# david8862/tf-keras-speech-commands

Measured on AMD Instinct MI355X. Metric: 1 s@16 kHz clips/sec train-step, simple_cnn bs4096, 1/2/4/8 MI355X; eval top-1, higher is better.
Workload: dtype f32; 1 GPU; configs[1]: simple_cnn train step = featurize(f32 1 s @16 kHz) + fwd + bwd + Adam, 36 logits (background + 35 words), batch 4096 per GPU; global_batch=4096, parallelism=dp1, gradient_exchange=none (one rank), rccl_ranks=0, library_build=ed8bfb18a7f8

## Files before the change

### tf-keras-speech-commands_amd/csrc/kws_cnn_shape.h

```cpp
#pragma once
#include <algorithm>
#include <cstddef>
#include <cstdint>

#include "kws.h"

namespace kws {

constexpr int kStatStride = 1024;
constexpr int kMaxStatBlocks = kStatStride;

constexpr int kFuClips = 16;
constexpr int kFuH2 = 7, kFuW2 = 5;
constexpr int kFuH3 = 4, kFuW3 = 3;
constexpr int kFuH4 = 2, kFuW4 = 1;
constexpr int kFuHeadCols = 48;
constexpr int kGrH1 = 2 * kFuH2 + 1, kGrW1 = 2 * kFuW2;

constexpr int kL1MaxTiles = 40;
constexpr int kL1Stage = 12;

constexpr int kDhK = 128;
constexpr int kDhWaves = 8;

// ... 41 lines not shown
    int pmajor = 0;
};

inline ConvGeom geom3x3(int B, int H, int W, int stride)
{
    ConvGeom g;
    g.B = B; g.H = H; g.W = W; g.stride = stride; g.KH = 3; g.KW = 3;
    g.Ho = same_out(H, stride); g.Wo = same_out(W, stride);
    g.pt = same_pad_before(H, 3, stride); g.pl = same_pad_before(W, 3, stride);
    return g;
}
inline ConvGeom geom1x1(int B, int H, int W)
{
    ConvGeom g;
    g.B = B; g.H = H; g.W = W; g.Ho = H; g.Wo = W; g.stride = 1; g.pt = 0; g.pl = 0; g.KH = 1; g.KW = 1;
    return g;
}
inline ConvGeom dense_geom(const CnnDims &d, int B)
{
    ConvGeom g;
    g.B = B; g.H = d.H4; g.W = d.W4; g.Ho = 1; g.Wo = 1; g.stride = 1; g.pt = 0; g.pl = 0; g.KH = d.H4; g.KW = d.W4;
    return g;
}

inline void stat_grid(long M, int C, int &nblk, int &rows)
{
    const int R = 256 / C;
    long want = (M + (long)R * 8 - 1) / ((long)R * 8);
    nblk = (int)std::min<long>(kMaxStatBlocks, std::max<long>(1, want));
    rows = (int)((M + nblk - 1) / nblk);
    nblk = (int)((M + rows - 1) / rows);
}

constexpr int conv_bf16_rt(bool fwd, int CR, int CO) { return (fwd && CO == 128 && CR == 64) ? 3 : 2; }
inline int conv_bf16_pmajor(const ConvGeom &g, bool fwd)
{
    const int P = fwd ? g.Ho * g.Wo : g.H * g.W;
    return (g.KH == 3 && g.KW == 3 && P > 1 && P <= 16) ? 1 : 0;
}

struct DgradClass { int cy, cx, ny, nx; };
struct DgradClasses { DgradClass c[4]; };

struct DgradPlan { DgradClasses cls; int ncls; long max_rows; int mw; };
enum { DGRAD_OK = 0, DGRAD_KERNEL_TOO_LARGE = 1, DGRAD_STRIDE = 2 };
inline int dgrad_plan(const ConvGeom &g, long simds, DgradPlan &p)
{
    if (g.KH > 8 * g.stride || g.KW > 8 * g.stride) return DGRAD_KERNEL_TOO_LARGE;
    DgradClasses &cls = p.cls;
    int ncls = 0;
    long rows[4] = {0, 0, 0, 0}, max_rows = 0;
    for (int cy = 0; cy < g.stride && cy < 2; ++cy)
        for (int cx = 0; cx < g.stride && cx < 2; ++cx) {
            DgradClass c{cy, cx, (g.H - cy + g.stride - 1) / g.stride, (g.W - cx + g.stride - 1) / g.stride};
            if (c.ny <= 0 || c.nx <= 0) continue;
            rows[ncls] = (long)g.B * c.ny * c.nx;
            max_rows = std::max(max_rows, rows[ncls]);
            cls.c[ncls++] = c;
        }
    for (int i = ncls; i < 4; ++i) cls.c[i] = DgradClass{0, 0, 0, 0};
    if (g.stride > 2) return DGRAD_STRIDE;
    int best = 4;
    long best_cost = -1;
    for (int mw = 4; mw >= 1; --mw) {
        long waves = 0;
        for (int i = 0; i < ncls; ++i) waves += ((rows[i] + 15) / 16 + mw - 1) / mw;
        const long cost = ((waves + simds - 1) / simds) * mw;
        if (best_cost < 0 || cost < best_cost) { best_cost = cost; best = mw; }
    }
    p.ncls = ncls; p.max_rows = max_rows; p.mw = best;
    return DGRAD_OK;
}

struct WgradRound { long gx; int spw; };
inline WgradRound wgrad_round(long steps, int gy, long resident, bool deterministic)
{
    const long slots = deterministic ? 1 : std::max<long>(1, resident / gy);
    const long gx_want = std::max<long>(1, std::min<long>(slots, (steps + 4 * 8 - 1) / (4 * 8)));
    const int spw = (int)((steps + 4 * gx_want - 1) / (4 * gx_want));
    const long gx = (steps + 4L * spw - 1) / (4L * spw);
    return WgradRound{gx, spw};
}

struct WgradBf16Round { long nranges; int cpb; };
inline WgradBf16Round wgrad_bf16_round(long nchunk, int ngroups, long resident, bool deterministic)
{
    long nranges = std::max<long>(8, (resident / ngroups) / 8 * 8);
    nranges = std::min<long>(nranges, std::max<long>(8, (nchunk / 4 + 7) / 8 * 8));
    int cpb = (int)((nchunk + nranges - 1) / nranges);
    if (deterministic) { nranges = 8; cpb = (int)nchunk; }
    return WgradBf16Round{nranges, cpb};
}

struct WgradPm {
    unsigned long long pos[9];
    int npos[9];
    int slot0[10];
};

inline bool wgrad_pm_plan(const ConvGeom &g, int max_slots, int min_chunks, WgradPm &pm)
{
    const int P = g.Ho * g.Wo, ntaps = g.KH * g.KW;
    if (P < 1 || P > 16 || ntaps < 1 || ntaps > 9) return false;
    long w[9], wsum = 0;
    int live = 0;
    for (int tap = 0; tap < ntaps; ++tap) {
        const int kh = tap / g.KW, kw = tap % g.KW;
        pm.pos[tap] = 0ull; pm.npos[tap] = 0;
        for (int p = 0; p < P; ++p) {
            const int sy = (p / g.Wo) * g.stride + kh - g.pt, sx = (p % g.Wo) * g.stride + kw - g.pl;
            if (sy < 0 || sy >= g.H || sx < 0 || sx >= g.W) continue;
            pm.pos[tap] |= (unsigned long long)p << (4 * pm.npos[tap]);
            ++pm.npos[tap];
        }
        w[tap] = pm.npos[tap]; wsum += w[tap]; live += w[tap] > 0;
    }
    if (live < 1 || max_slots < live) return false;
    const long nclip = ((long)g.B + 31) / 32, want = (wsum * nclip + 8L * min_chunks - 1) / (8L * min_chunks);
    const int S = (int)(want < live ? live : want > max_slots ? max_slots : want);
    int s[9], total = 0;
    for (int tap = 0; tap < ntaps; ++tap) {
        s[tap] = w[tap] ? (int)((long)S * w[tap] / wsum) : 0;
        if (w[tap] && s[tap] < 1) s[tap] = 1;
        total += s[tap];
    }
    for (; total < S; ++total) {
        int best = -1;
        for (int tap = 0; tap < ntaps; ++tap)
            if (w[tap] && (best < 0 || w[tap] * s[best] > w[best] * s[tap])) best = tap;
        ++s[best];
    }
    for (; total > S; --total) {
        int best = -1;
        for (int tap = 0; tap < ntaps; ++tap)
            if (s[tap] > 1 && (best < 0 || w[tap] * s[best] <= w[best] * s[tap])) best = tap;
        --s[best];
    }
    pm.slot0[0] = 0;
    for (int tap = 0; tap < ntaps; ++tap) pm.slot0[tap + 1] = pm.slot0[tap] + s[tap];
    for (int tap = ntaps + 1; tap < 10; ++tap) pm.slot0[tap] = pm.slot0[ntaps];
    return true;
}

struct L1Grid {
    int cpb, nb;
    int cpw, nbm;
};
inline L1Grid l1_grid(int B)
{
    L1Grid g;
    g.cpb = std::max(1, (B + kMaxStatBlocks - 1) / kMaxStatBlocks); g.nb = (B + g.cpb - 1) / g.cpb;
    g.cpw = std::max(1, (B + 4 * kMaxStatBlocks - 1) / (4 * kMaxStatBlocks)); g.nbm = (B + 4 * g.cpw - 1) / (4 * g.cpw);
    return g;
}

inline unsigned even_grid(int B, int max_blocks) { const int cpb = (B + max_blocks - 1) / max_blocks; return (unsigned)((B + cpb - 1) / cpb); }

struct LiteFrontGrid { int cpw, nblk; };
inline LiteFrontGrid lite_front_grid(int B, int cus, size_t sm)
{
    const int waves = cus * std::max(1, std::min(8, (int)(160 * 1024 / sm)));
    const int cpw = std::max(1, (B + waves - 1) / waves), nblk = (B + cpw - 1) / cpw;
    return LiteFrontGrid{cpw, nblk};
}

inline bool head_bwd_fuses(int K, int C) { return K % 16 == 0 && K <= 128 && C <= 48; }
// ... 3 lines not shown
```

### tf-keras-speech-commands_amd/csrc/kws_model.hip

```cpp
#include <cstdlib>
#include <cstring>
#include <string>
#include <type_traits>
#include <vector>

#include "kws_common.h"
#include "kws_model_types.h"
#include "kws_conv.h"
#include "kws_layers.h"
#include "kws_layer1.h"
#include "kws_layer1_moments.h"
#include "kws_layer1_fast.h"
#include "kws_l1_conv2.h"
#include "kws_conv2_wgrad_fast.h"
#include "kws_lite.h"
#include "kws_lite_f16.h"
#include "kws_infer_fused.h"
#include "kws_conv_group.h"
#include "kws_dense_head.h"
#include "kws_cnn_plan.h"

using namespace kws;

namespace {

struct OverlapHook {
    hipEvent_t ev = nullptr;
    void (*cb)(void *) = nullptr;
    void *user = nullptr;
    int at = 0;
    bool fired = false;
    bool wants(int point) const { return !fired && point == at; }
    int fire(int point, hipStream_t s, bool already_bound = false)
    {
        if (fired || point != at) return KWS_OK;
        fired = true;
        if (ev && !already_bound) KWS_HIP_CHECK(hipEventRecord(ev, s));
        if (cb) cb(user);
        return KWS_OK;
    }
};

#define KWS_TRY_NB(...)               \
    do {                              \
        const int rc__ = (__VA_ARGS__); \
        if (rc__ < 0) return rc__;    \
    } while (0)
#define KWS_TRY(...)                  \
    do {                              \
        if (int rc__ = (__VA_ARGS__)) return rc__; \
    } while (0)

inline CnnDesc cnn_desc(const kws_model *m) { return CnnDesc{m->kind, m->C, m->head_K, m->deterministic, m->d}; }

struct CnnWs {
    float *z[4], *a[4], *d1, *loss_i, *correct_i, *dlogits, *dd1, *da4, *gz[4], *da[3];
    float *dwo[4], *ddw[4];
    float *coef[4];
    __bf16 *wsp[3][6];
    __bf16 *dzp[3];
    double *partial;
    double *moments;
    float *zmax2;
    unsigned char *arg2;
    float *zmax4;
    unsigned char *arg4;
    unsigned char *base;
    size_t bytes;
};

CnnWs carve_cnn(const kws_model *m, int B, bool training, unsigned char *base)
{
    CnnWs w{};
    w.base = base;
    size_t off = 0;
    auto take = [&](size_t nfloats) {
        float *p = reinterpret_cast<float *>(base + off);
        off = al256(off + nfloats * sizeof(float));
        return p;
    };
    const CnnDims &d = m->d;
    const bool lite = m->kind == KWS_SIMPLE_CNN_LITE;
    size_t zs[4], as[4], dws[4];
    for (int i = 0; i < 4; ++i) {
        const CnnStage t = cnn_stage(d, i);
        zs[i] = (size_t)t.Ho * t.Wo * t.Cout;
        as[i] = t.pooled ? (size_t)(t.Ho / 2) * (t.Wo / 2) * t.Cout : zs[i];
        dws[i] = (size_t)t.Ho * t.Wo * t.Cin;
    }
    for (int i = 0; i < 4; ++i) { w.z[i] = take((i == 0 && !lite) ? 0 : zs[i] * B); w.a[i] = take(as[i] * B); }
    for (int i = 0; i < 4; ++i) w.dwo[i] = take(lite ? dws[i] * B : 0);
    w.d1 = take((size_t)B * 128);
    w.loss_i = take(B);
    w.correct_i = take(B);
    for (int i = 0; i < 4; ++i) w.coef[i] = take(6 * 128);
    {
        const size_t wn[3] = {(size_t)9 * 32 * 64, (size_t)9 * 64 * 128, (size_t)d.flat * 128};
        for (int t = 0; t < 3; ++t)
            for (int q = 0; q < 6; ++q) w.wsp[t][q] = reinterpret_cast<__bf16 *>(take(lite ? 0 : (wn[t] + 1) / 2));
    }
    w.partial = reinterpret_cast<double *>(take((size_t)kMaxStatBlocks * 9 * 64 * 2));
    w.moments = reinterpret_cast<double *>(take(2 * kMomCount));
    if (training) {
        w.dlogits = take((size_t)B * m->C);
        w.dd1 = take((size_t)B * 128);
        w.da4 = take((size_t)B * d.flat);
        for (int i = 0; i < 4; ++i) w.gz[i] = take((i == 0 && !lite) ? 0 : zs[i] * B);
        for (int p = 0; p < 3; ++p) w.dzp[p] = reinterpret_cast<__bf16 *>(take(lite ? 0 : (zs[3] * B + 1) / 2));
        for (int i = 0; i < 4; ++i) w.ddw[i] = take(lite ? dws[i] * B : 0);
        for (int i = 0; i < 3; ++i) w.da[i] = take(as[i] * B);
        w.zmax2 = take(lite ? 0 : as[1] * B);
        w.arg2 = reinterpret_cast<unsigned char *>(take(lite ? 0 : (as[1] * B + 3) / 4));
        w.zmax4 = take(lite ? 0 : as[3] * B);
        w.arg4 = reinterpret_cast<unsigned char *>(take(lite ? 0 : (as[3] * B + 3) / 4));
    }
    w.bytes = off;
    return w;
}

BnCoef coef_of(float *base, int C) { return BnCoef{base, base + C, base + 2 * C, base + 3 * C, base + 4 * C, base + 5 * C}; }
static double *acc_set(ModelRes *R, int pass, int layer, unsigned parity) { return R->acc + ((size_t)(pass * 4 + layer) * 2 + (parity & 1u)) * kAccDoubles; }
static int acc_make_clean(ModelRes *R, hipStream_t s)
{
    if (R->acc_dirty) {
        KWS_HIP_CHECK(hipMemsetAsync(R->acc, 0, sizeof(double) * 2 * 4 * 2 * kAccDoubles, s));
        R->acc_dirty = false;
    }
    return KWS_OK;
}

static int infer_coefs(const kws_model *m, const float *params, const float *state, CnnWs &w, hipStream_t s)
{
    BnInferAll a;
    for (int l = 0; l < 4; ++l) {
        a.C[l] = kCh[l + 1];
        a.gamma[l] = params + m->o_g[l]; a.beta[l] = params + m->o_b[l];
        a.mm[l] = state + m->o_mm[l]; a.mv[l] = state + m->o_mv[l];
        a.k[l] = coef_of(w.coef[l], kCh[l + 1]);
    }
    KWS_LAUNCH("bn_infer_coef_all_kernel", bn_infer_coef_all_kernel, dim3(4), dim3(128), 0, s, a);
    return KWS_OK;
}

template <int CR, int CO, int MODE, int EPI>
int launch_gemm(const float *src, const float *w, const float *bias, float *dst, const ConvGeom &g, hipStream_t s)
{
    const long M = (long)g.B * g.Ho * g.Wo;
    static const std::string name = std::string("conv_gemm_fwd<") + std::to_string(CR) + "," +
                                    std::to_string(CO) + ">";
    KWS_LAUNCH(name.c_str(), (conv_gemm_kernel<CR, CO, MODE, EPI>), dim3(blocks_for(M, 64)), dim3(256), 0, s, src, w, bias, dst, g);
    return KWS_OK;
}

static int cu_count() { return device_cus(); }
template <typename K>
static int resident_blocks(K kernel, int threads, size_t smem)
{
    int nb = 0;
    if (hipOccupancyMaxActiveBlocksPerMultiprocessor(&nb, kernel, threads, smem) != hipSuccess || nb < 1) { (void)hipGetLastError(); nb = 1; }
    return nb;
}

template <int CIN, int COUT, int GPB>
int launch_wgrad(const float *x, const float *dz, float *dw, const ConvGeom &g, hipStream_t s, bool deterministic = false,
                 const LossSumJob *job = nullptr)
{
    const float *zp = zero_page();
    if (!zp) return fail(KWS_ERR_NOMEM, "cannot allocate the zero page on this device");
    constexpr int CB = CIN >= 64 ? 64 : CIN;
    constexpr size_t smem = (4 * 64 * 4 + 16 * COUT) * sizeof(float);
    const long M = (long)g.B * g.Ho * g.Wo;
    const int ngroups = g.KH * g.KW * (CIN / CB), gy = (ngroups + GPB - 1) / GPB;
    const long steps = (M + 3) / 4;
    static const int occ = resident_blocks(conv_wgrad_direct_kernel<CIN, COUT, GPB>, 256, smem);
    const WgradRound r = wgrad_round(steps, gy, (long)cu_count() * occ, deterministic);
    static const std::string name = "conv_wgrad<" + std::to_string(CIN) + "," + std::to_string(COUT) + ">";
    KWS_LAUNCH(name.c_str(), (conv_wgrad_direct_kernel<CIN, COUT, GPB>), dim3((unsigned)r.gx + (job ? 1u : 0u), (unsigned)gy), dim3(256), smem,
               s, x, dz, dw, zp, g, r.spw, job ? *job : LossSumJob{});
    return KWS_OK;
}

template <int CIN, int COUT, int TPB, bool DPRE = false, bool XBN = false>
int launch_wgrad_bf16(const float *x, const float *dz, float *dw, const ConvGeom &g, hipStream_t s, __bf16 *const *dz_planes = nullptr,
                      bool deterministic = false, const float *xbn = nullptr, bool pmajor = false)
{
    if (TPB != 1 && g.KW != TPB) return fail(KWS_ERR_UNSUPPORTED, "split-precision weight gradient expects a kernel %d taps wide", TPB);
    const float *zp = zero_page();
    if (!zp) return fail(KWS_ERR_NOMEM, "cannot allocate the zero page on this device");
    constexpr size_t stage = (size_t)3 * 32 * 4 * (TPB * tr_row_words(CIN) + tr_row_words(COUT)), tile = (size_t)CIN * COUT * sizeof(float);
    constexpr size_t smem = stage > tile ? stage : tile;
    if (int rc = ensure_dynamic_lds(reinterpret_cast<const void *>(conv_wgrad_bf16_kernel<CIN, COUT, TPB, DPRE, XBN>), (int)smem)) return rc;
    static const int occ = resident_blocks(conv_wgrad_bf16_kernel<CIN, COUT, TPB, DPRE, XBN>, 256, smem);
    const long M = (long)g.B * g.Ho * g.Wo, nchunk = (M + 31) / 32;
    const int ngroups = g.KH * g.KW / TPB;
    const WgradBf16Round r = wgrad_bf16_round(nchunk, ngroups, (long)cu_count() * occ, deterministic);
    static const std::string name = "conv_wgrad_bf16<" + std::to_string(CIN) + "," + std::to_string(COUT) + ">";
    const Bf16Planes dpl{{DPRE ? dz_planes[0] : nullptr, DPRE ? dz_planes[1] : nullptr, DPRE ? dz_planes[2] : nullptr}};
    if (pmajor && TPB != 1) return fail(KWS_ERR_UNSUPPORTED, "the position-major weight gradient takes one tap per block");
    if constexpr (TPB == 1) {
        if (pmajor) {
            if (int rc = ensure_dynamic_lds(reinterpret_cast<const void *>(conv_wgrad_bf16_kernel<CIN, COUT, 1, DPRE, XBN, true>), (int)smem)) return rc;
            static const int occ_pm = resident_blocks(conv_wgrad_bf16_kernel<CIN, COUT, 1, DPRE, XBN, true>, 256, smem);
            WgradPm pm{};
            if (!wgrad_pm_plan(g, cu_count() * occ_pm / 8, 4, pm))
                return fail(KWS_ERR_UNSUPPORTED, "position-major weight gradient: a %d x %d map on %d block slots", g.Ho, g.Wo, cu_count() * occ_pm);
            KWS_LAUNCH(name.c_str(), (conv_wgrad_bf16_kernel<CIN, COUT, 1, DPRE, XBN, true>), dim3(8u * (unsigned)pm.slot0[ngroups]), dim3(256), smem, s, x,
                       dz, dw, zp, g, 0, 0, dpl, xbn, pm);
            return KWS_OK;
        }
    }
    KWS_LAUNCH(name.c_str(), (conv_wgrad_bf16_kernel<CIN, COUT, TPB, DPRE, XBN>), dim3((unsigned)(r.nranges * ngroups)), dim3(256), smem, s, x, dz, dw,
               zp, g, r.cpb, (int)r.nranges, dpl, xbn);
    return KWS_OK;
}

template <int CR, int CO, int MW, int STRIDE>
int launch_dgrad_mw(const float *dz, const float *w, float *dx, const ConvGeom &g, const DgradClasses &cls, int ncls, long max_rows,
                     hipStream_t s)
{
    static const std::string name = "conv_dgrad<" + std::to_string(CR) + "," + std::to_string(CO) + ">";
    const float *zp = zero_page();
    if (!zp) return fail(KWS_ERR_NOMEM, "cannot allocate the zero page on this device");
    KWS_LAUNCH(name.c_str(), (conv_dgrad_direct_kernel<CR, CO, MW, STRIDE>), dim3(blocks_for(max_rows, 64 * MW), (unsigned)ncls), dim3(256), 0, s,
               dz, w, dx, zp, g, cls);
    return KWS_OK;
}

template <int CR, int CO, int STRIDE>
int launch_dgrad(const float *dz, const float *w, float *dx, const ConvGeom &g, hipStream_t s)
{
    DgradPlan p;
    switch (dgrad_plan(g, 4L * cu_count(), p)) {
    case DGRAD_KERNEL_TOO_LARGE:
        return fail(KWS_ERR_UNSUPPORTED, "kernel %dx%d too large for the dgrad tap masks (at most %d taps per axis)", g.KH, g.KW, 8 * g.stride);
    case DGRAD_STRIDE: return fail(KWS_ERR_UNSUPPORTED, "dgrad is built for strides 1 and 2");
    default: break;
    }
    switch (p.mw) {
    case 1: return launch_dgrad_mw<CR, CO, 1, STRIDE>(dz, w, dx, g, p.cls, p.ncls, p.max_rows, s);
    case 2: return launch_dgrad_mw<CR, CO, 2, STRIDE>(dz, w, dx, g, p.cls, p.ncls, p.max_rows, s);
    case 3: return launch_dgrad_mw<CR, CO, 3, STRIDE>(dz, w, dx, g, p.cls, p.ncls, p.max_rows, s);
    default: return launch_dgrad_mw<CR, CO, 4, STRIDE>(dz, w, dx, g, p.cls, p.ncls, p.max_rows, s);
    }
}

static int g_matrix_precision = 1;
static inline int matrix_prec(const kws_model *m) { return m->matrix_precision >= 0 ? m->matrix_precision : g_matrix_precision; }
static int g_infer_precision = 0;
static inline int infer_prec(const kws_model *m) { return m->infer_precision >= 0 ? m->infer_precision : g_infer_precision; }

template <int CR, int CO, int MODE, int EPI>
int launch_bf16(const char *what, const float *src, __bf16 *const planes[6], const float *bias, float *dst, const ConvGeom &g_in,
                hipStream_t s, double *partial = nullptr, const float *shift = nullptr, __bf16 *const *src_planes = nullptr,
                const float *abn = nullptr)
{
    ConvGeom g = g_in;
    const long M = MODE == MODE_FWD ? (long)g.B * g.Ho * g.Wo : (long)g.B * g.H * g.W;
    if (M >= (1L << 31)) return fail(KWS_ERR_UNSUPPORTED, "%s: %ld rows exceed the kernel's 32-bit row index", what, M);
    g.pmajor = conv_bf16_pmajor(g, MODE == MODE_FWD);
    static const std::string name = std::string(what) + "<" + std::to_string(CR) + "," + std::to_string(CO) + ">";
    const int o = MODE == MODE_FWD ? 3 : 0;
    const Bf16Planes wp{{planes[o], planes[o + 1], planes[o + 2]}};
// ... 264 lines not shown
                       params + m->o_g[0], params + m->o_b[0], state + m->o_mm[0], state + m->o_mv[0], k1, w.a[0], B, d.H0, d.W0, g.cpw, g.nbm, pa);
        } else {
            KWS_LAUNCH("l1m_act_pool_kernel", l1m_act_pool_moments_kernel<false>, dim3(g.nbm), dim3(256), g.smemm, s, feat, kern1, q,
                       params + m->o_g[0], params + m->o_b[0], state + m->o_mm[0], state + m->o_mv[0], k1, w.a[0], B, d.H0, d.W0, g.cpw, g.nbm, pa);
        }
        return KWS_OK;
    }
    if (P.training) {
        KWS_LAUNCH("l1_stats_kernel", l1_stats_kernel<16>, dim3(g.nb), dim3(256), g.smem1, s, feat, kern1, B, d.H0, d.W0, g.cpb, w.partial);
        KWS_TRY(bn_train_coefs(0, g.nb));
    }
    if (P.l1m) KWS_LAUNCH("l1m_act_pool_kernel", l1m_act_pool_kernel, dim3(g.nbm), dim3(256), g.smemm, s, feat, kern1, k1.scale, k1.shift, w.a[0], B,
               d.H0, d.W0, g.cpw);
    else KWS_LAUNCH("l1_act_pool_kernel", l1_act_pool_kernel<16>, dim3(g.nb), dim3(256), g.smem1, s, feat, kern1, k1.scale, k1.shift, w.a[0], B,
               d.H0, d.W0, g.cpb);
    return KWS_OK;
}

int CnnStep::bn_train_coefs(int l, int fused_stat_blocks)
{
    const long M = pixels(l);
    const int C = kCh[l + 1];
    int nblk, rows;
    stat_grid(M, C, nblk, rows);
    if (fused_stat_blocks) nblk = fused_stat_blocks;
    else KWS_LAUNCH(prof_name("channel_stats_kernel", l + 1), channel_stats_kernel, dim3(nblk), dim3(256), 0, s, w.z[l], M, C, rows, w.partial);
    KWS_LAUNCH(prof_name("bn_finalize_train_kernel", l + 1), bn_finalize_train_kernel, dim3(C), dim3(64), 0, s, w.partial, nblk, M, C, params + m->o_g[l],
               params + m->o_b[l], state + m->o_mm[l], state + m->o_mv[l], coef(l));
    return KWS_OK;
}
int CnnStep::bn_act(int l, float rate, float *zm, unsigned char *ag)
{
    const BnCoef k = coef(l);
    const CnnStage t = cnn_stage(d, l);
    const int H = t.Ho, W = t.Wo, C = t.Cout;
    if (t.pooled) {
        const long total = (long)B * (H / 2) * (W / 2) * C;
        KWS_LAUNCH(prof_name("bn_act_pool_kernel", l + 1), bn_act_pool_kernel<true>, dim3(blocks_for(total, 256)), dim3(256), 0, s, w.z[l], k.scale, k.shift,
                   w.a[l], B, H, W, C, rate, slo(), shi(), zm, ag);
    } else {
        const long total = pixels(l) * C;
        KWS_LAUNCH(prof_name("bn_act_pool_kernel", l + 1), bn_act_pool_kernel<false>, dim3(blocks_for(total, 256)), dim3(256), 0, s, w.z[l], k.scale, k.shift,
                           w.a[l], B, H, W, C, rate, slo(), shi());
    }
    return KWS_OK;
}
int CnnStep::bn_bwd_finalize(int l, int nblk)
{
    const int C = kCh[l + 1];
    KWS_LAUNCH(prof_name("bn_bwd_finalize_kernel", l + 1), bn_bwd_finalize_kernel, dim3(C), dim3(64), 0, s, w.partial, nblk, pixels(l), C, params + m->o_g[l],
               grads + m->o_g[l], grads + m->o_b[l], coef(l));
    return KWS_OK;
}
template <bool RELU>
int CnnStep::bn_bwd_apply(int l)
{
    const int C = kCh[l + 1];
    const long total = pixels(l) * C;
    KWS_LAUNCH(prof_name("bn_bwd_apply_kernel", l + 1), bn_bwd_apply_kernel<RELU>, dim3(blocks_for(total, 256)), dim3(256), 0, s, w.z[l], w.gz[l], coef(l),
               params + m->o_g[l], total, C);
    return KWS_OK;
}

int CnnStep::colsum(const char *label, const float *x, long M, int C, float *dst)
{
    int nblk, rows;
    stat_grid(M, C, nblk, rows);
    KWS_LAUNCH(label, channel_stats_kernel, dim3(nblk), dim3(256), 0, s, x, M, C, rows, w.partial);
    KWS_LAUNCH("colsum_finalize_kernel", colsum_finalize_kernel, dim3(C), dim3(256), 0, s, w.partial, nblk, C, dst);
    return KWS_OK;
}
int CnnStep::head_train(const kws_train_args *a, float *stats)
{
    KWS_TRY(run_head(m, B, params, w.d1, w.loss_i, w.correct_i, a->labels, a->class_weights, a->probs, nullptr, w.dlogits, a->grad_scale / (float)B,
                     stats, a->ignore_index, s));
    if (a->forward_event) KWS_HIP_CHECK(hipEventRecord(static_cast<hipEvent_t>(a->forward_event), s));
    return KWS_OK;
}

int CnnStep::dense_fwd() { return launch_gemm<128, 128, MODE_FWD, EPI_BIAS_RELU6>(w.a[3], params + m->o_dk, params + m->o_db, w.d1, dense_geom(d, B), s); }
int CnnStep::dense_bias_grad() { return colsum("channel_stats_kernel.dense", w.dd1, B, 128, grads + m->o_db); }
int CnnStep::dense_wgrad(hipStream_t on, bool det, const LossSumJob *job)
{
    return launch_wgrad<128, 128, 1>(w.a[3], w.dd1, grads + m->o_dk, dense_geom(d, B), on, det, job);
}
int CnnStep::dense_dgrad() { return launch_dgrad<128, 128, 1>(w.dd1, params + m->o_dk, w.da4, dense_geom(d, B), s); }

int CnnCtx::fwd_conv2()
{
    const float *in = w.a[0], *kern = params + m->o_k[1];
    const unsigned nblk = (unsigned)std::min(B, kMaxStatBlocks);
    const Conv2Clip cc = conv2_clip(d, B);
    if (!P.training) {
        const BnCoef k2 = coef(1);
        if (P.bf16) {
            KWS_LAUNCH("conv_fwd_clip_pool_bf16<16,32>", (conv_fwd_clip_bf16_kernel<false, true>), dim3(nblk), dim3(256), cc.smb, s, in, kern, w.a[1], B,
                       d.H1, d.W1, w.partial, kStatStride, k2.scale, k2.shift);
            if (P.fused_tail) KWS_TRY(launch_fused_tail(m, B, params, w, probs, argmax, s));
        } else
            KWS_LAUNCH("conv_fwd_clip_pool<16,32>", (conv_fwd_clip_kernel<32, false, true>), dim3(nblk), dim3(256), cc.sm, s, in, kern, w.a[1], B,
                       d.H1, d.W1, w.partial, kStatStride, k2.scale, k2.shift);
        return KWS_OK;
    }
    if (P.l1_conv2) ;
    else if (P.bf16)
        KWS_LAUNCH("conv_fwd_clip_bf16<16,32>", (conv_fwd_clip_bf16_kernel<true>), dim3(nblk), dim3(256), cc.smb, s, in, kern, w.z[1], B, d.H1,
                   d.W1, w.partial, kStatStride, nullptr, nullptr, P.acc_fwd ? acc_set(R, 0, 1, fpar[1]) : nullptr);
    else
        KWS_LAUNCH("conv_fwd_clip<16,32>", (conv_fwd_clip_kernel<32, true>), dim3(nblk), dim3(256), cc.sm, s, in, kern, w.z[1], B, d.H1, d.W1,
                   w.partial, kStatStride);
    if (hook) KWS_TRY(hook->fire(9, s));
    if (!P.acc_fwd) KWS_TRY(bn_train_coefs(1, (int)nblk));
    if (!P.fuse_pool2) KWS_TRY(bn_act(1, 0.f, P.routed_g2 ? w.zmax2 : nullptr, P.routed_g2 ? w.arg2 : nullptr));
    return KWS_OK;
}

int CnnCtx::fwd_conv3()
{
    const float *in = w.a[1], *kern = params + m->o_k[2];
    const ConvGeom g = geom3x3(B, d.H2, d.W2, 2);
    if (P.bf16 && !P.training) {
        const BnCoef k3 = coef(2);
        KWS_TRY_NB(launch_bf16<32, 64, MODE_FWD, EPI_BN_RELU6>("conv_bf16_fwd_bn", in, w.wsp[0], k3.scale, w.a[2], g, s, nullptr, k3.shift));
        return KWS_OK;
    }
    if (P.bf16 && P.training && !P.prep_in_stats) KWS_HIP_CHECK(hipStreamWaitEvent(s, R->ev[11], 0));
    int fused_stat_blocks = 0;
    if (P.group) {
        if (P.acc_fwd) { const BnAccFwd in2 = acc_in(1, fpar[1]); fused_stat_blocks = launch_group_conv3(m, B, w, s, P.fuse_pool2, &in2, acc_set(R, 0, 2, fpar[2])); }
        else fused_stat_blocks = launch_group_conv3(m, B, w, s, P.fuse_pool2);
        if (fused_stat_blocks < 0) return fused_stat_blocks;
    } else if (P.bf16) {
        fused_stat_blocks = launch_bf16<32, 64, MODE_FWD, EPI_NONE>("conv_bf16_fwd", in, w.wsp[0], nullptr, w.z[2], g, s, P.training ? w.partial : nullptr);
        if (fused_stat_blocks < 0) return fused_stat_blocks;
    } else KWS_TRY(launch_gemm<32, 64, MODE_FWD, EPI_NONE>(in, kern, nullptr, w.z[2], g, s));
    if (hook) KWS_TRY(hook->fire(10, s));
    if (P.training && !P.acc_fwd) KWS_TRY(bn_train_coefs(2, fused_stat_blocks));
    if (!P.a3_on_load) KWS_TRY(bn_act(2, 0.f));
    return KWS_OK;
}

int CnnCtx::fwd_conv4()
{
    const float *in = w.a[2], *kern = params + m->o_k[3];
    const ConvGeom g = geom3x3(B, d.H3, d.W3, 1);
    int fused_stat_blocks = 0;
    if (P.group) {
        if (P.acc_fwd) { const BnAccFwd in3 = acc_in(2, fpar[2]); fused_stat_blocks = launch_group_conv4(m, B, w, s, &in3, acc_set(R, 0, 3, fpar[3])); }
        else fused_stat_blocks = launch_group_conv4(m, B, w, s);
        if (fused_stat_blocks < 0) return fused_stat_blocks;
    } else if (P.bf16) {
        fused_stat_blocks = launch_bf16<64, 128, MODE_FWD, EPI_RELU>("conv_bf16_fwd", P.a3_on_load ? w.z[2] : in, w.wsp[1], nullptr, w.z[3], g, s,
                                                                   P.training ? w.partial : nullptr, nullptr, nullptr,
                                                                   P.a3_on_load ? coef(2).scale : nullptr);
        if (fused_stat_blocks < 0) return fused_stat_blocks;
    } else KWS_TRY(launch_gemm<64, 128, MODE_FWD, EPI_RELU>(in, kern, nullptr, w.z[3], g, s));
    if (P.training && !P.acc_fwd) KWS_TRY(bn_train_coefs(3, fused_stat_blocks));
    const float rate = P.training ? drop_rate() : 0.f;
    if (hook) KWS_TRY(hook->fire(0, s));
    if (P.pool4_fused) return KWS_OK;
    const bool arm6 = hook && hook->wants(6) && hook->ev;
    if (arm6) arm_stop_event(hook->ev, s);
    float *zm = P.training && P.bf16 ? w.zmax4 : nullptr;
    unsigned char *ag = P.training && P.bf16 ? w.arg4 : nullptr;
    if (P.acc_fwd) {
        const long total = (long)B * (d.H3 / 2) * (d.W3 / 2) * 128;
// ... 153 lines not shown
}

int CnnCtx::bwd_layer3()
{
    const int C = 64, H = d.H3, W = d.W3;
    if (hook) KWS_TRY(hook->fire(5, s));
    const long M = pixels(2);
    const BnCoef k = coef(2);
    const float *gamma = params + m->o_g[2];
    int nblk, rows;
    stat_grid(M, C, nblk, rows);
    if (fused_bn3_blocks > 0) nblk = fused_bn3_blocks;
    else
        KWS_LAUNCH(prof_name("bn_bwd_reduce_kernel", 3), bn_bwd_reduce_kernel<false>, dim3(nblk), dim3(256), 0, s, w.z[2], w.da[2], k, w.gz[2], B, H, W, C,
                   rows, w.partial, 0.f, slo(), shi());
    if (!P.acc_bn3) KWS_TRY(bn_bwd_finalize(2, nblk));
    bwd_arm(2);
    if (P.acc_bn3)
        KWS_LAUNCH(prof_name("bn_bwd_apply_kernel", 3), bn_bwd_apply_acc_kernel<false>, dim3(std::min<unsigned>(1024u, blocks_for(M * C / 4, 256))), dim3(256), 0, s,
                   w.z[2], w.gz[2], k, gamma, M * C / 4, C, acc_out(2));
    else KWS_TRY(bn_bwd_apply<false>(2));
    KWS_TRY(bwd_fork(2));
    const float *in = w.a[1], *kern = params + m->o_k[2];
    float *dk = grads + m->o_k[2];
    const ConvGeom g = geom3x3(B, d.H2, d.W2, 2);
    if (P.bf16) KWS_TRY(launch_wgrad_bf16<32, 64, 3>(in, w.gz[2], dk, g, s2, nullptr, P.det));
    else KWS_TRY(launch_wgrad<32, 64, 3>(in, w.gz[2], dk, g, s2, P.det));
    if (P.group) {
        if (P.acc_bn2) bwd_arm(1);
        KWS_TRY(launch_group_dgrad3(m, B, w, s, P.acc_bn2 ? acc_set(R, 1, 1, bpar[1]) : nullptr));
    }
    else KWS_TRY(launch_dgrad<64, 32, 2>(w.gz[2], kern, w.da[1], g, s));
    return KWS_OK;
}

int CnnCtx::bwd_layer2()
{
    const int C = 32, H1 = d.H1, W1 = d.W1;
    const long M = pixels(1);
    const BnCoef k = coef(1);
    const long NW = (long)B * (H1 / 2) * (W1 / 2);
    int nblk, rows;
    stat_grid(NW, C, nblk, rows);
    if (P.acc_bn2) ;
    else if (P.compact_g2 && P.routed_g2)
        KWS_LAUNCH(prof_name("bn_bwd_reduce_pool_kernel", 2), bn_bwd_reduce_routed_kernel, dim3(nblk), dim3(256), 0, s, w.zmax2, w.da[1], k, NW, C,
                   rows, w.partial);
    else if (P.compact_g2)
        KWS_LAUNCH(prof_name("bn_bwd_reduce_pool_kernel", 2), bn_bwd_reduce_pool_kernel<true>, dim3(nblk), dim3(256), 0, s, w.z[1], w.da[1], k,
                   w.gz[1], B, H1, W1, C, rows, w.partial, 0.f, slo(), shi(), reinterpret_cast<unsigned char *>(w.da[2]));
    else KWS_TRY(bwd_reduce_pool(1, H1, W1, C, w.da[1], 0.f, nblk, rows));
    if (!P.acc_bn2) {
        if (P.wgrad2_early) bwd_arm(1);
        KWS_TRY(bn_bwd_finalize(1, nblk));
    }
    const float *in = w.a[0], *kern = params + m->o_k[1];
    float *dk = grads + m->o_k[1];
    const Conv2Clip cc = conv2_clip(d, B);
    BnBwdArgs bn = {w.z[1], params + m->o_g[1], k.mean, k.inv, k.k2, k.k3};
    if (P.compact_g2) { bn.gw = w.da[1]; bn.arg = P.routed_g2 ? w.arg2 : reinterpret_cast<const unsigned char *>(w.da[2]); }
    BnBwdArgs bn_w = bn;
    if (P.acc_bn2) {
        bn.acc = bn_w.acc = acc_set(R, 1, 1, bpar[1]);
        bn.M = bn_w.M = M;
        bn.acc_clear_set = acc_set(R, 1, 1, bpar[1] + 1);
        bn.dgamma = grads + m->o_g[1]; bn.dbeta = grads + m->o_b[1]; bn.k2w = k.k2; bn.k3w = k.k3;
    }
    auto wgrad_grid = [&](int occ) { return dim3(P.det ? 1u : cc.even_grid(cu_count() * std::min(occ, 2))); };
    if (P.wgrad2_early) {
        KWS_TRY(bwd_fork(1));
        arm_stop_event(R->ev[9], s2);
        if (P.wgrad2_fast) {
            using G = Conv2WgradFast<kW2fH, kW2fW>;
            if (int rc = ensure_dynamic_lds(reinterpret_cast<const void *>(conv2_wgrad_fast_kernel<kW2fH, kW2fW>), G::BYTES)) return rc;
            KWS_LAUNCH("conv_wgrad_clip_bf16<16,32>", (conv2_wgrad_fast_kernel<kW2fH, kW2fW>), dim3(G::grid(B, cu_count() * 2)), dim3(256), G::BYTES, s2, in, dk,
                       B, bn_w);
        } else {
            static const int occ = resident_blocks(conv_wgrad_clip_bf16_kernel<true>, 256, cc.smwb);
            KWS_LAUNCH("conv_wgrad_clip_bf16<16,32>", conv_wgrad_clip_bf16_kernel<true>, wgrad_grid(occ), dim3(256), cc.smwb, s2, in, nullptr, dk, B, H1, W1, bn_w);
        }
    }
    if (P.bf16) {
        const dim3 grid(cc.even_grid(cu_count() * 2));
        if (P.wgrad2_early)
            KWS_LAUNCH("conv_dgrad_clip_bf16<32,16>", (conv_dgrad_clip_bf16_kernel<true, true, false>), grid, dim3(256), cc.smdb, s,
                       w.gz[1], kern, w.da[0], B, H1, W1, bn);
        else if (P.compact_g2)
            KWS_LAUNCH("conv_dgrad_clip_bf16<32,16>", (conv_dgrad_clip_bf16_kernel<true, true>), grid, dim3(256), cc.smdb, s,
                       w.gz[1], kern, w.da[0], B, H1, W1, bn);
        else
            KWS_LAUNCH("conv_dgrad_clip_bf16<32,16>", (conv_dgrad_clip_bf16_kernel<true, false>), grid, dim3(256), cc.smdb, s,
                       w.gz[1], kern, w.da[0], B, H1, W1, bn);
    } else
        KWS_LAUNCH("conv_dgrad_clip<32,16>", (conv_dgrad_clip_kernel<32, true>), dim3(cc.even_grid(cu_count() * 5)), dim3(256), cc.smd, s, w.gz[1], kern, w.da[0],
                   B, H1, W1, bn);
    if (P.wgrad2_early) return KWS_OK;
    KWS_TRY(bwd_fork(1));
    if (P.wgrad2_bf16) {
        static const int occ = resident_blocks(conv_wgrad_clip_bf16_kernel<false>, 256, cc.smwb);
        KWS_LAUNCH("conv_wgrad_clip_bf16<16,32>", conv_wgrad_clip_bf16_kernel<false>, wgrad_grid(occ), dim3(256), cc.smwb, s2, in, w.gz[1], dk, B, H1, W1, bn);
    } else
        KWS_LAUNCH("conv_wgrad_clip<16,32>", conv_wgrad_clip_kernel<32>, dim3(P.det ? 1u : cc.even_grid(cu_count() * 3)), dim3(256), cc.smw, s2, in, w.gz[1], dk,
                   B, H1, W1);
    return KWS_OK;
}

int CnnCtx::bwd_layer1()
{
    const L1Geom g = l1_geom(d, B, P);
    BnCoef k1 = coef(0);
    const float *kern1 = params + m->o_k[0];
    if (P.l1m) {
        const double *q = moments ? moments : w.moments;
        if (P.l1_fin_in_kernel) {
            double *acc0 = acc_set(R, 1, 0, 0);
            const L1FinalizeArgs fin{acc0, reinterpret_cast<unsigned *>(acc0 + kAccDoubles - 1), q, params + m->o_g[0], grads + m->o_k[0],
                                     grads + m->o_g[0], grads + m->o_b[0]};
            KWS_LAUNCH("l1m_bwd_onepass_kernel", (l1f_bwd_onepass_kernel<30, 20>), dim3(g.nbm), dim3(256), g.smemm, s, feat, kern1, w.da[0], k1, B, g.cpw, w.partial, fin);
        } else if (P.l1_default_map)
            KWS_LAUNCH("l1m_bwd_onepass_kernel", (l1f_bwd_onepass_kernel<30, 20>), dim3(g.nbm), dim3(256), g.smemm, s, feat, kern1, w.da[0], k1, B, g.cpw, w.partial);
        else
            KWS_LAUNCH("l1m_bwd_onepass_kernel", l1m_bwd_onepass_kernel, dim3(g.nbm), dim3(256), g.smemm, s, feat, kern1, w.da[0], k1, B, d.H0, d.W0, g.cpw,
                       w.partial);
        if (!P.l1_fin_in_kernel)
            KWS_LAUNCH("l1_bwd_finalize_moments_kernel", l1_bwd_finalize_moments_kernel, dim3(144 + 16), dim3(64), 0, s, w.partial, g.nbm, q, kern1,
                       params + m->o_g[0], k1, grads + m->o_k[0], grads + m->o_g[0], grads + m->o_b[0]);
    } else {
        KWS_LAUNCH("l1_bwd_reduce_kernel", l1_bwd_reduce_kernel<16>, dim3(g.nb), dim3(256), g.smem1, s, feat, kern1, w.da[0], k1, B, d.H0, d.W0,
                   g.cpb, w.partial);
        KWS_TRY(bn_bwd_finalize(0, g.nb));
        KWS_LAUNCH("l1_bwd_wgrad_kernel", l1_bwd_wgrad_kernel<16>, dim3(P.det ? 1 : g.nb), dim3(256), g.smem1, s, feat, kern1, w.da[0], k1, params + m->o_g[0],
                   grads + m->o_k[0], B, d.H0, d.W0, P.det ? B : g.cpb);
    }
    return KWS_OK;
}

int CnnCtx::backward()
{
    const DisarmOnExit disarm_guard;
    if (!P.bf16) KWS_HIP_CHECK(hipMemsetAsync(grads, 0, sizeof(float) * (size_t)m->P, s));
    bpar[1] = P.acc_bn2 ? R->acc_uses[1][1]++ : 0u;
    bpar[2] = P.acc_bn3 ? R->acc_uses[1][2]++ : 0u;
    bpar[3] = P.acc_bn4 ? R->acc_uses[1][3]++ : 0u;
    KWS_TRY(acc_make_clean(R, s));
    R->acc_dirty = true;
    KWS_TRY(bwd_head_dense());
    KWS_TRY(bwd_layer4());
    KWS_TRY(bwd_layer3());
    KWS_TRY(bwd_layer2());
    KWS_TRY(bwd_layer1());
    if (!stop_event_bound(R->ev[9])) KWS_HIP_CHECK(hipEventRecord(R->ev[9], s2));
    KWS_HIP_CHECK(hipStreamWaitEvent(s, R->ev[9], 0));
    KWS_LAUNCH_CHECK("simple_cnn backward");
    R->acc_dirty = false;
    return KWS_OK;
}


struct LiteCtx : CnnStep {
    bool det;
    int forward(bool training);
    int forward_f16(float *probs, int32_t *argmax);
    int backward(hipEvent_t bucket_event);
    int fwd_stage(int l, bool training), bwd_stage(int l);
};

template <typename F>
// ... 654 lines not shown
```

### tf-keras-speech-commands_amd/csrc/kws_cnn_plan.h

```cpp
#pragma once
#include "kws_cnn_shape.h"

namespace kws {

struct CnnPlan {
    bool training, bf16, det;
    bool prepared;
    bool fused_tail;
    bool group;
    bool dense_fused;
    bool l1m;
    bool l1_default_map;
    bool prep_in_stats;
    bool l1_conv2;
    bool compact_g2;
    bool routed_g2;
    bool fuse_pool2;
    bool acc_fwd;
    bool acc_bn2, acc_bn3, acc_bn4;
    bool a3_on_load;
    bool pool4_fused;
    bool wgrad_pmajor;
    bool wgrad2_bf16;
    bool wgrad2_early;
    bool wgrad2_fast;
    bool l1_fin_in_kernel;
    bool head_bwd_fuses;
    bool fuse_head_fwd;
};

struct CnnDesc { int kind, C, head_K, deterministic; CnnDims d; };

inline CnnPlan plan_cnn(const CnnDesc &m, int B, int mprec, bool training, bool capturing, bool wants_head_outputs, bool prepared)
{
    const CnnDims &d = m.d;
    CnnPlan p{};
    p.training = training;
    p.bf16 = mprec == 1;
    p.det = m.deterministic != 0;
    p.prepared = !training && prepared;
    const bool split_train = p.bf16 && training;
    const bool default_tail = m.kind == KWS_SIMPLE_CNN && d.H2 == kFuH2 && d.W2 == kFuW2 && d.H3 == kFuH3 && d.W3 == kFuW3;
    p.fused_tail = !training && wants_head_outputs && p.bf16 && default_tail && d.H4 == kFuH4 && d.W4 == kFuW4 && m.C <= kFuHeadCols;
    p.group = split_train && default_tail && (long)blocks_for(B, kFuClips) <= kStatStride;
    p.head_bwd_fuses = head_bwd_fuses(m.head_K, m.C);
    p.fuse_head_fwd = p.head_bwd_fuses && !p.det;
    p.dense_fused = split_train && m.kind == KWS_SIMPLE_CNN && p.fuse_head_fwd && m.head_K == kDhK && d.flat % (16 * kDhWaves) == 0 && d.flat <= 1024;
    p.l1m = d.H0 % 2 == 0 && d.W0 % 2 == 0 && (d.H0 + 2) * (d.W0 + 2) <= 64 * kL1Stage && (d.H0 / 2) * (d.W0 / 2) <= 4 * kL1MaxTiles;
    p.l1_default_map = d.H0 == 30 && d.W0 == 20;
    p.prep_in_stats = split_train && p.l1m;
    const int P1 = d.H1 * d.W1;
    p.compact_g2 = p.bf16 && P1 * 8 <= 1280 && (size_t)(d.H1 / 2) * (d.W1 / 2) * 32 <= sizeof(float) * (size_t)d.H3 * d.W3 * 64;
    p.routed_g2 = p.compact_g2;
    p.fuse_pool2 = p.group && p.routed_g2 && d.H1 == kGrH1 && d.W1 == kGrW1;
    const bool acc_ok = !p.det && !capturing;
    p.acc_fwd = p.fuse_pool2 && acc_ok;
    p.l1_conv2 = p.prep_in_stats && p.acc_fwd && p.l1_default_map;
    p.a3_on_load = split_train;
    p.pool4_fused = p.acc_fwd && p.dense_fused;
    p.wgrad_pmajor = split_train && !p.det && d.H3 * d.W3 <= 16;
    p.wgrad2_bf16 = p.bf16 && P1 <= 160;
    p.wgrad2_early = p.compact_g2 && p.wgrad2_bf16 && P1 * 8 <= 1280 && P1 * 4 <= 768;
    p.acc_bn2 = p.group && acc_ok && p.routed_g2 && p.wgrad2_early;
    p.acc_bn3 = p.group && acc_ok;
    p.acc_bn4 = p.dense_fused && acc_ok && d.flat == d.H4 * d.W4 * kDhK;
    p.l1_fin_in_kernel = acc_ok && p.l1_default_map;
    p.wgrad2_fast = p.wgrad2_early && p.acc_bn2 && d.H1 == kW2fH && d.W1 == kW2fW;
    return p;
}

}
```

Before: 8.180 million clips/s.

## Add dedicated split-K MFMA kernel for dense layer weight gradient

```diff
diff --git a/tf-keras-speech-commands_amd/csrc/kws_cnn_shape.h b/tf-keras-speech-commands_amd/csrc/kws_cnn_shape.h
--- a/tf-keras-speech-commands_amd/csrc/kws_cnn_shape.h
+++ b/tf-keras-speech-commands_amd/csrc/kws_cnn_shape.h
@@ -147,6 +147,22 @@
     return WgradRound{gx, spw};
 }
 
+constexpr int kDwTile = 64, kDwMinSteps = 8;
+struct DenseWgradGrid { int tm, tn, nranges, spr; };
+inline bool dense_wgrad_grid(int B, int flat, int units, int cus, long resident, DenseWgradGrid &g)
+{
+    if (B < 1 || flat < kDwTile || units < kDwTile || flat % kDwTile || units % kDwTile) return false;
+    if ((long)B * std::max(flat, units) >= (1L << 31)) return false;
+    const long tiles = (long)(flat / kDwTile) * (units / kDwTile), slots = std::min<long>(cus, resident - 1);
+    if (slots < tiles) return false;
+    const long steps = ((long)B + 3) / 4;
+    const long want = std::max<long>(1, std::min<long>(slots / tiles, steps / kDwMinSteps));
+    g.tm = flat / kDwTile; g.tn = units / kDwTile;
+    g.spr = (int)((steps + want - 1) / want);
+    g.nranges = (int)((steps + g.spr - 1) / g.spr);
+    return true;
+}
+
 struct WgradBf16Round { long nranges; int cpb; };
 inline WgradBf16Round wgrad_bf16_round(long nchunk, int ngroups, long resident, bool deterministic)
 {
diff --git a/tf-keras-speech-commands_amd/csrc/kws_dense_wgrad.h b/tf-keras-speech-commands_amd/csrc/kws_dense_wgrad.h
--- /dev/null
+++ b/tf-keras-speech-commands_amd/csrc/kws_dense_wgrad.h
@@ -0,0 +1,84 @@
+#pragma once
+#include "kws_cnn_shape.h"
+#include "kws_device.h"
+
+namespace kws {
+
+constexpr int kDwDepth = 16;
+constexpr int kDwRow = kDwTile + 4;
+
+__global__ __launch_bounds__(256) void dense_wgrad_kernel(const float *__restrict__ x, const float *__restrict__ dz, float *__restrict__ dw,
+                                                          const float *__restrict__ zeros, int B, int flat, int units, DenseWgradGrid grid,
+                                                          LossSumJob job)
+{
+    __shared__ __attribute__((aligned(16))) float red[kDwTile * kDwRow];
+    const int tiles = grid.tm * grid.tn, nblk = tiles * grid.nranges;
+    if ((int)blockIdx.x >= nblk) {
+        if (job.out) loss_sum_block(job.loss_i, job.correct_i, job.B, job.out, reinterpret_cast<double *>(red));
+        return;
+    }
+    int tile, range;
+    if (grid.nranges % 8 == 0) {
+        const int q = (int)blockIdx.x >> 3;
+        tile = q % tiles;
+        range = (q / tiles) * 8 + ((int)blockIdx.x & 7);
+    } else {
+        tile = (int)blockIdx.x % tiles;
+        range = (int)blockIdx.x / tiles;
+    }
+    const int lane = threadIdx.x & 63, wave = threadIdx.x >> 6, li = lane & 15, lq = lane >> 4;
+    const int wm = wave >> 1, wn = wave & 1;
+    const int row0 = kDwTile * (tile / grid.tn), col0 = kDwTile * (tile % grid.tn);
+    const int step0 = range * grid.spr;
+    const int left = (B + 3) / 4 - step0, nst = left < grid.spr ? left : grid.spr;
+
+    const int xo = row0 + 32 * wm + 2 * li, dzo = col0 + 32 * wn + 2 * li;
+    auto load_frags = [&](float2 &af, float2 &bf, int st) {
+        const int clip = 4 * (step0 + st) + lq;
+        const bool ok = st < nst && clip < B;
+        af = *reinterpret_cast<const float2 *>(ok ? x + (clip * flat + xo) : zeros + 2 * li);
+        bf = *reinterpret_cast<const float2 *>(ok ? dz + (clip * units + dzo) : zeros + 2 * li);
+    };
+
+    f32x4 acc[2][2];
+#pragma unroll
+    for (int em = 0; em < 2; ++em)
+#pragma unroll
+        for (int en = 0; en < 2; ++en) acc[em][en] = (f32x4){0.f, 0.f, 0.f, 0.f};
+
+    float2 afr[kDwDepth], bfr[kDwDepth];
+#pragma unroll
+    for (int i = 0; i < kDwDepth; ++i) load_frags(afr[i], bfr[i], i);
+    asm volatile("" ::: "memory");
+    for (int s0 = 0; s0 < nst; s0 += kDwDepth) {
+#pragma unroll
+        for (int i = 0; i < kDwDepth; ++i) {
+            const float2 af = afr[i], bf = bfr[i];
+            acc[0][0] = mfma16(af.x, bf.x, acc[0][0]);
+            acc[0][1] = mfma16(af.x, bf.y, acc[0][1]);
+            acc[1][0] = mfma16(af.y, bf.x, acc[1][0]);
+            acc[1][1] = mfma16(af.y, bf.y, acc[1][1]);
+            load_frags(afr[i], bfr[i], s0 + kDwDepth + i);
+            asm volatile("" ::: "memory");
+        }
+    }
+
+#pragma unroll
+    for (int em = 0; em < 2; ++em)
+#pragma unroll
+        for (int r = 0; r < 4; ++r)
+            *reinterpret_cast<float2 *>(&red[(32 * wm + 2 * (4 * lq + r) + em) * kDwRow + 32 * wn + 2 * li]) = make_float2(acc[em][0][r], acc[em][1][r]);
+    __syncthreads();
+    float *out = dw + (long)row0 * units + col0;
+#pragma unroll
+    for (int j = 0; j < kDwTile * kDwTile / 256; ++j) {
+        const int idx = (int)threadIdx.x + 256 * j, row = idx / kDwTile, col = idx % kDwTile;
+#if defined(KWS_EXP_DW_NO_ATOMICS)
+        out[row * units + col] = red[row * kDwRow + col];
+#else
+        atomicAdd(out + row * units + col, red[row * kDwRow + col]);
+#endif
+    }
+}
+
+}
diff --git a/tf-keras-speech-commands_amd/csrc/kws_model.hip b/tf-keras-speech-commands_amd/csrc/kws_model.hip
--- a/tf-keras-speech-commands_amd/csrc/kws_model.hip
+++ b/tf-keras-speech-commands_amd/csrc/kws_model.hip
@@ -18,6 +18,7 @@
 #include "kws_infer_fused.h"
 #include "kws_conv_group.h"
 #include "kws_dense_head.h"
+#include "kws_dense_wgrad.h"
 #include "kws_cnn_plan.h"
 
 using namespace kws;
@@ -178,6 +179,17 @@
     KWS_LAUNCH(name.c_str(), (conv_wgrad_direct_kernel<CIN, COUT, GPB>), dim3((unsigned)r.gx + (job ? 1u : 0u), (unsigned)gy), dim3(256), smem,
                s, x, dz, dw, zp, g, r.spw, job ? *job : LossSumJob{});
     return KWS_OK;
+}
+
+static bool launch_dense_wgrad(const float *x, const float *dz, float *dw, int B, int flat, int units, hipStream_t s, const LossSumJob *job)
+{
+    const float *zp = zero_page();
+    static const int occ = resident_blocks(dense_wgrad_kernel, 256, 0);
+    DenseWgradGrid g;
+    if (!zp || !dense_wgrad_grid(B, flat, units, cu_count(), (long)cu_count() * occ, g)) return false;
+    KWS_LAUNCH("conv_wgrad<128,128>", dense_wgrad_kernel, dim3((unsigned)(g.tm * g.tn * g.nranges) + (job ? 1u : 0u)), dim3(256), 0, s, x, dz, dw, zp, B,
+               flat, units, g, job ? *job : LossSumJob{});
+    return true;
 }
 
 template <int CIN, int COUT, int TPB, bool DPRE = false, bool XBN = false>
@@ -608,6 +620,7 @@
 int CnnStep::dense_bias_grad() { return colsum("channel_stats_kernel.dense", w.dd1, B, 128, grads + m->o_db); }
 int CnnStep::dense_wgrad(hipStream_t on, bool det, const LossSumJob *job)
 {
+    if (!det && launch_dense_wgrad(w.a[3], w.dd1, grads + m->o_dk, B, d.flat, kDhK, on, job)) return KWS_OK;
     return launch_wgrad<128, 128, 1>(w.a[3], w.dd1, grads + m->o_dk, dense_geom(d, B), on, det, job);
 }
 int CnnStep::dense_dgrad() { return launch_dgrad<128, 128, 1>(w.dd1, params + m->o_dk, w.da4, dense_geom(d, B), s); }
```

After: 8.217 million clips/s (median of 4 runs). No clear change (+0.5%).

## Add specialized conv2 dgrad kernel fusing BN-backward and pool routing

Applied to the files above, without the earlier changes.

```diff
diff --git a/tf-keras-speech-commands_amd/csrc/kws_cnn_plan.h b/tf-keras-speech-commands_amd/csrc/kws_cnn_plan.h
--- a/tf-keras-speech-commands_amd/csrc/kws_cnn_plan.h
+++ b/tf-keras-speech-commands_amd/csrc/kws_cnn_plan.h
@@ -27,6 +27,7 @@
     bool l1_fin_in_kernel;
     bool head_bwd_fuses;
     bool fuse_head_fwd;
+    bool dgrad2_fast;
 };
 
 struct CnnDesc { int kind, C, head_K, deterministic; CnnDims d; };
@@ -66,6 +67,7 @@
     p.acc_bn4 = p.dense_fused && acc_ok && d.flat == d.H4 * d.W4 * kDhK;
     p.l1_fin_in_kernel = acc_ok && p.l1_default_map;
     p.wgrad2_fast = p.wgrad2_early && p.acc_bn2 && d.H1 == kW2fH && d.W1 == kW2fW;
+    p.dgrad2_fast = p.wgrad2_fast;
     return p;
 }
 
diff --git a/tf-keras-speech-commands_amd/csrc/kws_conv2_dgrad_fast.h b/tf-keras-speech-commands_amd/csrc/kws_conv2_dgrad_fast.h
--- /dev/null
+++ b/tf-keras-speech-commands_amd/csrc/kws_conv2_dgrad_fast.h
@@ -0,0 +1,170 @@
+#pragma once
+#include "kws_cnn_shape.h"
+
+namespace kws {
+
+template <int H, int W>
+struct Conv2DgradFast {
+    static constexpr int CR = 32, CO = 16, F4 = CR / 4, HP = H + 2, WP = W + 2, HW = H * W;
+    static constexpr int NPIX = (HP * WP + 15) & ~15, NTILE = (HW + 15) / 16;
+    static constexpr int QUARTER = NPIX * 16, PLANE = 4 * QUARTER, BYTES = 3 * PLANE;
+    static constexpr int HPL = H / 2, WPL = W / 2, NWIN = HPL * WPL;
+    static constexpr int WIN1 = 256 / F4;
+    static constexpr int LEFT = (NWIN - WIN1) * 4;
+    static constexpr int SLOTS = LEFT + (H - 2 * HPL) * W;
+    static constexpr int SPW = (SLOTS + 3) / 4;
+    static_assert(W % 2 == 0, "every column lies in a pool window");
+    static_assert(NWIN >= WIN1 && SPW * F4 <= 64, "one window unit per thread, then at most one pixel per thread");
+    static_assert(BYTES % 16 == 0 && BYTES <= 64 * 1024, "the planes fit the default dynamic LDS limit");
+};
+
+template <int H, int W>
+__global__ __launch_bounds__(256, 2) void conv2_dgrad_fast_kernel(const float *__restrict__ wgt, float *__restrict__ dx, int B, BnBwdArgs bn)
+{
+    using G = Conv2DgradFast<H, W>;
+    constexpr int CR = G::CR, CO = G::CO, F4 = G::F4, WP = G::WP, HW = G::HW, NTILE = G::NTILE, WPL = G::WPL, NWIN = G::NWIN;
+    constexpr int QUARTER = G::QUARTER, PLANE = G::PLANE;
+    extern __shared__ __attribute__((aligned(16))) unsigned char ctile[];
+    const int lane = threadIdx.x & 63, wave = __builtin_amdgcn_readfirstlane(threadIdx.x >> 6), li = lane & 15, lq = lane >> 4;
+    for (int i = threadIdx.x; i < G::BYTES / 16; i += 256) reinterpret_cast<f32x4 *>(ctile)[i] = (f32x4){0.f, 0.f, 0.f, 0.f};
+
+    bf16x8 wf[9][3];
+#pragma unroll
+    for (int t = 0; t < 9; ++t) {
+        const f32x4 w0 = *reinterpret_cast<const f32x4 *>(wgt + (t * CO + li) * CR + 8 * lq);
+        const f32x4 w1 = *reinterpret_cast<const f32x4 *>(wgt + (t * CO + li) * CR + 8 * lq + 4);
+        bf16x4 h0, m0, l0, h1, m1, l1;
+        split_bf16(w0, h0, m0, l0);
+        split_bf16(w1, h1, m1, l1);
+        wf[t][0] = __builtin_shufflevector(h0, h1, 0, 1, 2, 3, 4, 5, 6, 7);
+        wf[t][1] = __builtin_shufflevector(m0, m1, 0, 1, 2, 3, 4, 5, 6, 7);
+        wf[t][2] = __builtin_shufflevector(l0, l1, 0, 1, 2, 3, 4, 5, 6, 7);
+    }
+
+    __shared__ __attribute__((aligned(16))) float coef[5][CR];
+    const int c4 = threadIdx.x & (F4 - 1);
+    {
+        f32x4 gi, mean, inv;
+        float k2[4], k3[4];
+#pragma unroll
+        for (int e = 0; e < 4; ++e) {
+            const int c = 4 * c4 + e;
+            inv[e] = bn.inv[c]; gi[e] = bn.gamma[c] * inv[e]; mean[e] = bn.mean[c];
+        }
+        bn_bwd_k_from_acc(bn, CR, c4, bn.dgamma && blockIdx.x == 0, k2, k3);
+        if (bn.acc_clear_set && blockIdx.x == 0) acc_clear(bn.acc_clear_set, threadIdx.x, 256);
+        if (threadIdx.x < F4) {
+            *reinterpret_cast<f32x4 *>(&coef[0][4 * c4]) = gi;
+            *reinterpret_cast<f32x4 *>(&coef[1][4 * c4]) = mean;
+            *reinterpret_cast<f32x4 *>(&coef[2][4 * c4]) = inv;
+            *reinterpret_cast<f32x4 *>(&coef[3][4 * c4]) = (f32x4){k2[0], k2[1], k2[2], k2[3]};
+            *reinterpret_cast<f32x4 *>(&coef[4][4 * c4]) = (f32x4){k3[0], k3[1], k3[2], k3[3]};
+        }
+    }
+
+    const int wy = (int)(threadIdx.x >> 3) / WPL, wx = (int)(threadIdx.x >> 3) % WPL;
+    const int lds_c = (c4 >> 1) * QUARTER + (c4 & 1) * 8;
+    const int zo1 = (2 * wy * W + 2 * wx) * F4 + c4;
+    const int d1 = ((2 * wy + 1) * WP + 2 * wx + 1) * 16 + lds_c;
+    int zo2 = 0, d2 = -1, q2 = 0, ce2 = 0x100;
+    {
+        const int sl = wave * G::SPW + (lane >> 3);
+        if (lane < G::SPW * F4 && sl < G::SLOTS) {
+            int y, x;
+            if (sl < G::LEFT) {
+                const int win = G::WIN1 + sl / 4, e = sl % 4;
+                y = 2 * (win / WPL) + (e >> 1); x = 2 * (win % WPL) + (e & 1);
+                q2 = win * F4 + c4; ce2 = e;
+            } else {
+                y = 2 * G::HPL + (sl - G::LEFT) / W; x = (sl - G::LEFT) % W;
+            }
+            zo2 = (y * W + x) * F4 + c4;
+            d2 = ((y + 1) * WP + x + 1) * 16 + lds_c;
+        }
+    }
+
+    struct Raw { f32x4 z[5], g[2]; unsigned a[2]; };
+    auto prefetch = [&](int b, Raw &r) {
+        const f32x4 *zs = reinterpret_cast<const f32x4 *>(bn.z) + (long)b * HW * F4;
+        const f32x4 *gws = reinterpret_cast<const f32x4 *>(bn.gw) + (long)b * NWIN * F4;
+        const unsigned *ars = reinterpret_cast<const unsigned *>(bn.arg) + (long)b * NWIN * F4;
+        r.g[0] = gws[threadIdx.x];
+        r.a[0] = ars[threadIdx.x];
+#pragma unroll
+        for (int e = 0; e < 4; ++e) r.z[e] = zs[zo1 + ((e >> 1) * W + (e & 1)) * F4];
+        r.g[1] = gws[q2];
+        r.a[1] = ars[q2];
+        r.z[4] = zs[zo2];
+    };
+    auto put = [&](int d, f32x4 v) {
+        bf16x4 h, m, l;
+        split_bf16(v, h, m, l);
+        *reinterpret_cast<bf16x4 *>(ctile + d) = h;
+        *reinterpret_cast<bf16x4 *>(ctile + d + PLANE) = m;
+        *reinterpret_cast<bf16x4 *>(ctile + d + 2 * PLANE) = l;
+    };
+    auto stage = [&](const Raw &r) {
+        const f32x4 gi = *reinterpret_cast<const f32x4 *>(&coef[0][4 * c4]), mean = *reinterpret_cast<const f32x4 *>(&coef[1][4 * c4]),
+                    inv = *reinterpret_cast<const f32x4 *>(&coef[2][4 * c4]), k2 = *reinterpret_cast<const f32x4 *>(&coef[3][4 * c4]),
+                    k3 = *reinterpret_cast<const f32x4 *>(&coef[4][4 * c4]);
+        auto dz2 = [&](f32x4 gw, unsigned aw, int ce, f32x4 zv) {
+            f32x4 v;
+#pragma unroll
+            for (int e = 0; e < 4; ++e) {
+                const float g = (int)((aw >> (8 * e)) & 0xFFu) == ce ? gw[e] : 0.f;
+                v[e] = gi[e] * (g - k2[e] - (zv[e] - mean[e]) * inv[e] * k3[e]);
+            }
+            return v;
+        };
+#pragma unroll
+        for (int e = 0; e < 4; ++e) put(d1 + ((e >> 1) * WP + (e & 1)) * 16, dz2(r.g[0], r.a[0], e, r.z[e]));
+        if (d2 >= 0) put(d2, dz2(r.g[1], r.a[1], ce2, r.z[4]));
+    };
+    constexpr int AHEAD = 2, RING = AHEAD + 1;
+    static_assert(9 % RING == 0, "the ring position of tap 0 is the same in every tile");
+    auto products = [&](int b, int t0) {
+        auto origin = [&](int t) {
+            const int p = 16 * t + li, pc = p < HW ? p : HW - 1;
+            const int ih = pc / W, iw = pc - ih * W;
+            return ctile + lq * QUARTER + ((ih + 2) * WP + iw + 2) * 16;
+        };
+        bf16x8 a[RING][3];
+        auto read = [&](const unsigned char *a0, int tap, bf16x8 (&f)[3]) {
+#pragma unroll
+            for (int pl = 0; pl < 3; ++pl) f[pl] = *reinterpret_cast<const bf16x8 *>(a0 - ((tap / 3) * WP + tap % 3) * 16 + pl * PLANE);
+        };
+        const unsigned char *a0 = origin(t0);
+#pragma unroll
+        for (int tap = 0; tap < AHEAD; ++tap) read(a0, tap, a[tap % RING]);
+        for (int t = t0; t < NTILE; t += 4) {
+            const unsigned char *an = origin(t + 4 < NTILE ? t + 4 : t);
+            f32x4 acc = {0.f, 0.f, 0.f, 0.f};
+#pragma unroll
+            for (int tap = 0; tap < 9; ++tap) {
+                if (tap + AHEAD < 9) read(a0, tap + AHEAD, a[(tap + AHEAD) % RING]);
+                else read(an, tap + AHEAD - 9, a[(tap + AHEAD) % RING]);
+                constexpr int pa[6] = {1, 2, 0, 1, 0, 0}, pb[6] = {1, 0, 2, 0, 1, 0};
+#pragma unroll
+                for (int i = 0; i < 6; ++i) acc = mfma_bf16(wf[tap][pb[i]], a[tap % RING][pa[i]], acc);
+                __builtin_amdgcn_sched_barrier(0);
+            }
+            const int po = 16 * t + li;
+            if (po < HW) *reinterpret_cast<f32x4 *>(dx + ((long)b * HW + po) * CO + 4 * lq) = acc;
+            a0 = an;
+        }
+    };
+
+    const int stride = gridDim.x;
+    int rot = wave;
+    Raw r;
+    if ((int)blockIdx.x < B) prefetch(blockIdx.x, r);
+    for (int b = blockIdx.x; b < B; b += stride, ++rot) {
+        __syncthreads();
+        stage(r);
+        __syncthreads();
+        if (b + stride < B) prefetch(b + stride, r);
+        products(b, rot & 3);
+    }
+}
+
+}
diff --git a/tf-keras-speech-commands_amd/csrc/kws_model.hip b/tf-keras-speech-commands_amd/csrc/kws_model.hip
--- a/tf-keras-speech-commands_amd/csrc/kws_model.hip
+++ b/tf-keras-speech-commands_amd/csrc/kws_model.hip
@@ -13,6 +13,7 @@
 #include "kws_layer1_fast.h"
 #include "kws_l1_conv2.h"
 #include "kws_conv2_wgrad_fast.h"
+#include "kws_conv2_dgrad_fast.h"
 #include "kws_lite.h"
 #include "kws_lite_f16.h"
 #include "kws_infer_fused.h"
@@ -927,7 +928,10 @@
     }
     if (P.bf16) {
         const dim3 grid(cc.even_grid(cu_count() * 2));
-        if (P.wgrad2_early)
+        if (P.dgrad2_fast) {
+            using G = Conv2DgradFast<kW2fH, kW2fW>;
+            KWS_LAUNCH("conv_dgrad_clip_bf16<32,16>", (conv2_dgrad_fast_kernel<kW2fH, kW2fW>), grid, dim3(256), G::BYTES, s, kern, w.da[0], B, bn);
+        } else if (P.wgrad2_early)
             KWS_LAUNCH("conv_dgrad_clip_bf16<32,16>", (conv_dgrad_clip_bf16_kernel<true, true, false>), grid, dim3(256), cc.smdb, s,
                        w.gz[1], kern, w.da[0], B, H1, W1, bn);
         else if (P.compact_g2)
```

Measured after the change: 8.263 million clips/s before, 8.447 million clips/s after, median of 6. 1.02x the previous value.
